# Lcrypto/mod-interleaveavx_multithreads-FAID

Measured on AMD Instinct MI355X. Metric: decoded Gb/s @ 10 iters, 50G-PON LDPC; FER match vs AVX512 ref, higher is better.
Workload: dtype i8

## Files before the change

include/lnsfaid.h:

```cpp
#ifndef LNSFAID_H
#define LNSFAID_H

#include <stddef.h>
#include <stdint.h>

#ifdef __cplusplus
extern "C" {
#endif

#define LNSFAID_GROUP 32

#define LNSFAID_OK 0
#define LNSFAID_E_INVAL (-1)
#define LNSFAID_E_CODE (-2)
#define LNSFAID_E_NOMEM (-3)
#define LNSFAID_E_HIP (-4)
#define LNSFAID_E_NODEVICE (-5)
#define LNSFAID_E_INTERNAL (-6)

typedef struct lnsfaid_code {
    int32_t n_var;
    int32_t n_check;
    int32_t n_edges;
    int32_t z;
// ... 215 lines not shown
int lnsfaid_select_kernel(lnsfaid_ctx* ctx, int32_t rows_per_lane);
int lnsfaid_kernel_rows_per_lane(const lnsfaid_ctx* ctx);

int lnsfaid_select_waves(lnsfaid_ctx* ctx, int32_t waves_per_codeword);
int lnsfaid_kernel_waves(const lnsfaid_ctx* ctx);

#define LNSFAID_MSG_REGISTERS 1
#define LNSFAID_MSG_HBM 2
int lnsfaid_select_message_store(lnsfaid_ctx* ctx, int32_t where);
int lnsfaid_message_store(const lnsfaid_ctx* ctx);

#define LNSFAID_ZERO_SHIFT_ON 1
#define LNSFAID_ZERO_SHIFT_OFF 2
#define LNSFAID_ZERO_SHIFT_LOOP 3
#define LNSFAID_ZERO_SHIFT_STATIC 4
int lnsfaid_select_zero_shift(lnsfaid_ctx* ctx, int32_t mode);
int lnsfaid_zero_shift_groups(const lnsfaid_ctx* ctx, int32_t* groups, int32_t n);
int lnsfaid_code_zero_shift_order(const lnsfaid_code* code, int32_t* groups, int32_t* order);

int lnsfaid_code_bf_walk(const lnsfaid_code* code, int32_t col_weight, uint32_t* full, uint32_t* flipped, uint32_t* fixed, int32_t* info);

int lnsfaid_kernel_residency(lnsfaid_ctx* ctx, int32_t* workgroups_per_cu, int32_t* lds_limit);


int lnsfaid_kernel_time(lnsfaid_ctx* ctx, double* out_ms, uint64_t* out_launches, int32_t reset);

void* lnsfaid_stream(lnsfaid_ctx* ctx);

const char* lnsfaid_strerror(int err);
const char* lnsfaid_last_hip_error(void);
const char* lnsfaid_version(void);

// ... 5 lines not shown
```

mod-interleaveavx_multithreads-faid_amd/csrc/lnsfaid_capi.hip:

```cpp
#include <hip/hip_runtime.h>

#include <dlfcn.h>
#include <rccl/rccl.h>

#include <cstdio>
#include <cstdlib>
#include <cstring>
#include <new>
#include <vector>

#include "lnsfaid_device.h"
#include "lnsfaid_line.h"
#include "lnsfaid_quantise.h"
#include "lnsfaid_swar.h"

extern "C" hipError_t lf_launch_decode(int method, int uniform_w, const LfKernelArgs* args, size_t lds_bytes,
                                       hipStream_t stream);
extern "C" const void* lf_decode_func(int method, int uniform_w);
extern "C" int lf_decode_threads(void);
extern "C" const void* lf_decode4_func(int method, int ef, int rm);
extern "C" int lf_decode4_threads(void);
extern "C" hipError_t lf_launch_decode4(int method, int ef, int rm, const LfKernelArgs* args, size_t lds_bytes, hipStream_t stream);
extern "C" int lf_decode4_rm_layers(void);
extern "C" const void* lf_decode4cw_func(int method, int ef, int rm);
// ... 1 lines not shown
extern "C" const void* lf_decode4p_func(int method, int ef, int rm, int per_codeword);
extern "C" hipError_t lf_launch_decode4p(int method, int ef, int rm, const LfKernelArgs* args, size_t lds_bytes, hipStream_t stream);
extern "C" hipError_t lf_launch_decode4pcw(int method, int ef, int rm, const LfCwArgs* args, size_t lds_bytes, hipStream_t stream);
extern "C" const void* lf_decode4l_func(int method, int ef, int rm);
extern "C" hipError_t lf_launch_decode4l(int method, int ef, int rm, const LfLineArgs* args, size_t lds_bytes, hipStream_t stream);
extern "C" hipError_t lf_launch_unpack_llr4(const uint8_t* d_llr4, int8_t* d_fix, size_t n_values, hipStream_t stream);
extern "C" hipError_t lf_launch_pack_bits(const int8_t* d_decoded, uint32_t* d_bits, size_t n_values, hipStream_t stream);
extern "C" hipError_t lf_launch_count_errors_packed(const uint32_t* d_bits, const uint32_t* d_msg, int n_var, int k_info, size_t n_cw,
                                                    unsigned long long* out, hipStream_t stream);
extern "C" int lf_decode4z_inst(int deg, int zg);
extern "C" const void* lf_decode4z_func(int method);
extern "C" hipError_t lf_launch_decode4z(int method, const LfKernelArgs* args, size_t lds_bytes, hipStream_t stream);
extern "C" int lf_decode4s_matches(const LfDevCode* code);
extern "C" const void* lf_decode4s_func(int method);
extern "C" hipError_t lf_launch_decode4s(int method, const LfKernelArgs* args, size_t lds_bytes, hipStream_t stream);
extern "C" const void* lf_decode5_func(int method);
extern "C" int lf_decode5_threads(void);
extern "C" hipError_t lf_launch_decode5(int method, const LfKernelArgs* args, size_t lds_bytes, hipStream_t stream);
extern "C" hipError_t lf_launch_count_errors(const int8_t* decoded, const int8_t* input_bits, int n_var, int k_info,
                                             size_t n_cw, unsigned long long* out, hipStream_t stream);

extern "C" hipError_t lf_launch_frontend(const uint32_t* d_seeds, const unsigned long long* d_draws, int n_streams, int mod_type,
                                         float sigma_ch, float scale, const int8_t* d_codeword, const int8_t* d_frames, int n_var,
                                         int n_check, int interleave, int fast, int8_t* d_fix, int count_limit,
                                         unsigned long long* d_frame_cnt, hipStream_t stream);
extern "C" hipError_t lf_launch_prefec(const float* d_rx, const int8_t* d_sent, size_t n_groups, int mod_type, int n_var, int n_check,
                                       int interleave, int scope, unsigned long long* d_out, hipStream_t stream);
extern "C" hipError_t lf_launch_prefec_fold(unsigned long long* d_frame_cnt, size_t n_streams, unsigned long long* d_acc, hipStream_t stream);
extern "C" hipError_t lf_launch_capture(const int8_t* d_fix, const int8_t* d_decoded, const int8_t* d_sent, size_t n_groups, int n_var,
                                        int n_check, uint32_t skip, uint32_t cap, uint2* d_cnt, uint32_t* d_slots,
// ... 435 lines not shown
    if (!out || !code || !cfg || max_groups == 0 || max_groups > ((size_t)1 << 24)) return LNSFAID_E_INVAL;
    *out = nullptr;
    lnsfaid_ctx* ctx = new (std::nothrow) lnsfaid_ctx();
    if (!ctx) return LNSFAID_E_NOMEM;
    ctx->device = device;
    ctx->max_groups = max_groups;
    if (const char* e = getenv("LNSFAID_ROWS_PER_LANE"))
        ctx->rows_per_lane = (e[0] == '2') ? 2 : 0;
    if (const char* e = getenv("LNSFAID_WAVES_PER_CODEWORD"))
        ctx->waves_per_cw = (e[0] == '2') ? 2 : 0;
    if (const char* e = getenv("LNSFAID_FRONTEND_EXACT"))
        ctx->fe_exact = (e[0] == '1') ? 1 : 0;
    if (const char* e = getenv("LNSFAID_MSG_STORE"))
        ctx->msg_store = (e[0] == 'h') ? LNSFAID_MSG_HBM : ((e[0] == 'r') ? LNSFAID_MSG_REGISTERS : 0);
    if (const char* e = getenv("LNSFAID_ZERO_SHIFT"))
        ctx->zero_shift = (e[0] == 'o' && e[1] == 'f') ? LNSFAID_ZERO_SHIFT_OFF : (e[0] == 'l' ? LNSFAID_ZERO_SHIFT_LOOP : 0);
    g_live_contexts.fetch_add(1, std::memory_order_relaxed);
    const int rc = create_impl(ctx, code, cfg);
    if (rc) { lnsfaid_destroy(ctx); return rc; }
    ctx->comb_slot = comb_join(ctx);
    *out = ctx;
    return LNSFAID_OK;
}

extern "C" int lnsfaid_set_cfg(lnsfaid_ctx* ctx, const lnsfaid_cfg* cfg)
{
    if (!ctx || !cfg) return LNSFAID_E_INVAL;
    LfDevCfg n;
    int rc = build_cfg(cfg, &n);
    if (rc) return rc;
    rc = check_code_for_method(&ctx->hcode, n.method);
// ... 79 lines not shown
    for (int br = 0; br < ctx->hcode.nbr; ++br)
        if (layer_zero_groups(ctx, br) >= 1) return true;
    return false;
}
static bool use_zero_shift(const lnsfaid_ctx* ctx) { return ctx->zero_shift != LNSFAID_ZERO_SHIFT_OFF && zero_shift_possible(ctx); }

static bool static_layers_possible(const lnsfaid_ctx* ctx)
{
    if (ctx->static_code < 0) ctx->static_code = lf_decode4s_matches(&ctx->hcode);
    return ctx->static_code == 1 && zero_shift_possible(ctx) && lf_decode4s_func(ctx->hcfg.method);
}
static bool use_static_layers(const lnsfaid_ctx* ctx)
{
    return use_zero_shift(ctx) && ctx->zero_shift != LNSFAID_ZERO_SHIFT_LOOP && static_layers_possible(ctx);
}

extern "C" int lnsfaid_select_zero_shift(lnsfaid_ctx* ctx, int32_t mode)
{
    if (!ctx || mode < 0 || mode > LNSFAID_ZERO_SHIFT_STATIC) return LNSFAID_E_INVAL;
    if ((mode == LNSFAID_ZERO_SHIFT_ON || mode == LNSFAID_ZERO_SHIFT_LOOP) && !zero_shift_possible(ctx)) return LNSFAID_E_INVAL;
    if (mode == LNSFAID_ZERO_SHIFT_STATIC && !static_layers_possible(ctx)) return LNSFAID_E_INVAL;
    ctx->zero_shift = mode;
    return LNSFAID_OK;
}

extern "C" int lnsfaid_zero_shift_groups(const lnsfaid_ctx* ctx, int32_t* groups, int32_t n)
{
    if (!ctx || n < 0 || (n > 0 && !groups)) return LNSFAID_E_INVAL;
    const bool on = use_zero_shift(ctx);
    for (int br = 0; br < n; ++br) groups[br] = (on && br < ctx->hcode.nbr) ? layer_zero_groups(ctx, br) : 0;
    return on ? (use_static_layers(ctx) ? 2 : 1) : 0;
}

extern "C" int lnsfaid_code_zero_shift_order(const lnsfaid_code* code, int32_t* groups, int32_t* order)
{
    LfDevCode* dc = new (std::nothrow) LfDevCode;
    if (!dc) return LNSFAID_E_NOMEM;
    const int rc = build_code(code, dc);
    if (rc) { delete dc; return rc; }
    const int nbr = dc->nbr;
    for (int br = 0; br < nbr; ++br) {
        int n_zero = 0;
        while (n_zero < dc->deg[br] && dc->zs4tab[br][n_zero] == 0u) ++n_zero;
        if (groups) groups[br] = n_zero / 4;
        for (int j = 0; order && j < LF_MAX_DEG; ++j) {
            order[br * LF_MAX_DEG + j] = -1;
// ... 43 lines not shown
{
    if (packed) {
        *threads = lf_decode4_threads();
        return lf_decode4p_func(ctx->hcfg.method, ctx->hcfg.ef, use_msg_registers(ctx) ? 1 : 0, rule == LNSFAID_STOP_CODEWORD ? 1 : 0);
    }
    if (rule == LNSFAID_STOP_CODEWORD) {
        *threads = lf_decode4_threads();
        return cw_possible(ctx) ? lf_decode4cw_func(ctx->hcfg.method, ctx->hcfg.ef, use_msg_registers(ctx) ? 1 : 0) : nullptr;
    }
    if (use_kernel5(ctx)) {
        *threads = lf_decode5_threads();
        return lf_decode5_func(ctx->hcfg.method);
    }
    if (use_zero_shift(ctx)) {
        *threads = lf_decode4_threads();
        return use_static_layers(ctx) ? lf_decode4s_func(ctx->hcfg.method) : lf_decode4z_func(ctx->hcfg.method);
    }
    if (use_kernel4(ctx)) {
        *threads = lf_decode4_threads();
        return lf_decode4_func(ctx->hcfg.method, ctx->hcfg.ef, use_msg_registers(ctx) ? 1 : 0);
    }
    *threads = lf_decode_threads();
    return lf_decode_func(ctx->hcfg.method, ctx->hcfg.uniform_w);
}

extern "C" int lnsfaid_select_message_store(lnsfaid_ctx* ctx, int32_t where)
{
    if (!ctx || where < 0 || where > LNSFAID_MSG_HBM) return LNSFAID_E_INVAL;
    if (where == LNSFAID_MSG_REGISTERS && !msg_registers_possible(ctx)) return LNSFAID_E_INVAL;
    ctx->msg_store = where;
// ... 142 lines not shown
    int cur = 0;
    long launch = 0, needed = 0;
    bool done = false;
    while (!done) {
        if (launch >= max_launches) return LNSFAID_E_INTERNAL;
        int chain = launch == 0 ? ctx->predicted_launches : 1;
        if (chain < 1) chain = 1;
        if (chain > LF_MAX_CHAIN) chain = LF_MAX_CHAIN;
        for (int j = 0; j < chain; ++j) {
            a.status_cur = (launch + j == 0 && !status_preloaded) ? nullptr : ctx->d_status[cur];
            a.status_next = ctx->d_status[cur ^ 1];
            a.remaining = ctx->d_remaining + j;
            HIP_TRY(hipEventRecord(ctx->ev_chain[j], ctx->stream));
            if (packed) HIP_TRY(lf_launch_decode4p(ctx->hcfg.method, ctx->hcfg.ef, use_msg_registers(ctx) ? 1 : 0, &a, ctx->lds_bytes, ctx->stream));
            else if (use_kernel5(ctx)) HIP_TRY(lf_launch_decode5(ctx->hcfg.method, &a, ctx->lds_bytes, ctx->stream));
            else if (use_static_layers(ctx)) HIP_TRY(lf_launch_decode4s(ctx->hcfg.method, &a, ctx->lds_bytes, ctx->stream));
            else if (use_zero_shift(ctx)) HIP_TRY(lf_launch_decode4z(ctx->hcfg.method, &a, ctx->lds_bytes, ctx->stream));
            else if (use_kernel4(ctx)) HIP_TRY(lf_launch_decode4(ctx->hcfg.method, ctx->hcfg.ef, use_msg_registers(ctx) ? 1 : 0, &a, ctx->lds_bytes, ctx->stream));
            else HIP_TRY(lf_launch_decode(ctx->hcfg.method, ctx->hcfg.uniform_w, &a, ctx->lds_bytes, ctx->stream));
            cur ^= 1;
        }
        HIP_TRY(hipEventRecord(ctx->ev_chain[chain], ctx->stream));
        HIP_TRY(hipMemcpyAsync(ctx->h_remaining, ctx->d_remaining, (size_t)chain * sizeof(uint32_t), hipMemcpyDeviceToHost, ctx->stream));
        { const int rcw = stream_wait(ctx); if (rcw) return rcw; }
        for (int j = 0; j < chain; ++j) {
            const uint32_t left = ctx->h_remaining[j] - ctx->slot_seen[j];
            ctx->slot_seen[j] = ctx->h_remaining[j];
            float ms = 0.f;
            HIP_TRY(hipEventElapsedTime(&ms, ctx->ev_chain[j], ctx->ev_chain[j + 1]));
            ctx->kernel_ms += ms;
// ... 1620 lines not shown
```

mod-interleaveavx_multithreads-faid_amd/csrc/lnsfaid_swar.h:

```cpp
#ifndef LNSFAID_SWAR_H
#define LNSFAID_SWAR_H

#include <stdint.h>

#if defined(__HIPCC__)
#define SW_DEV 1
#define SW_FN __device__ __forceinline__
#define SW_HD __host__ __device__ __forceinline__
#else
#define SW_DEV 0
#define SW_FN static inline
#define SW_HD static inline
#endif

#define SW_MAX_DEG 24
#ifndef SW_ILP
#define SW_ILP 4
#endif

#if SW_DEV
#define SW_SCHED_FENCE() __builtin_amdgcn_sched_barrier(0)
#else
#define SW_SCHED_FENCE() ((void)0)
#endif
// ... 60 lines not shown
    return k;
#endif
}

#define SW_T2N_LO 0xf900fafbu
#define SW_T2N_HI 0xf8000000u

struct SwK {
    uint32_t c78, c0642, cfc, sel_sign, tt_lo, tt_hi, oh_lo, oh_hi;
    uint32_t cbit[8];
    uint32_t c7f;
    uint32_t c70;
    uint32_t n_lo, n_hi;
    uint32_t c55, c33, c0f;
    uint32_t cm27;
};
SW_FN SwK sw_consts(uint32_t dep = 0u)
{
    SwK k;
    k.c78 = sw_vconst(0x78787878u, dep); k.c0642 = sw_vconst(0x06040200u, dep); k.cfc = sw_vconst(0xfcu, dep);
    k.sel_sign = sw_vconst(0x0b090a08u, dep);
    k.tt_lo = sw_vconst(0x07030100u, dep); k.tt_hi = sw_vconst(0xff3f1f0fu, dep);
    k.oh_lo = sw_vconst(0x08040201u, dep); k.oh_hi = sw_vconst(0x80402010u, dep);
    for (int e = 0; e < 8; ++e) k.cbit[e] = sw_vconst(0x01010101u << e, dep);
    k.c7f = sw_vconst(0x7f7f7f7fu, dep);
    k.c70 = sw_vconst(0x70707070u, dep);
    k.n_lo = sw_vconst(SW_T2N_LO, dep); k.n_hi = sw_vconst(SW_T2N_HI, dep);
    k.c55 = sw_vconst(0x55555555u, dep); k.c33 = sw_vconst(0x33333333u, dep); k.c0f = sw_vconst(0x0f0f0f0fu, dep);
    k.cm27 = sw_vconst(0u - 0x27272727u, dep);
    return k;
}

SW_FN uint32_t sw_mask7(uint32_t x, uint32_t sel_sign) { return sw_perm(x, x << 8, sel_sign); }
#define SW_SEL_SIGN 0x0b090a08u
SW_FN uint64_t sw_shl8x2(uint32_t& a, uint32_t& b)
{
    uint64_t p = ((uint64_t)b << 32) | a;
#if SW_DEV
    asm("" : "+v"(p));
    a = (uint32_t)p; b = (uint32_t)(p >> 32);
    uint64_t r = p << 8;
    asm("" : "+v"(r));
    return r;
#else
// ... 8 lines not shown
    *ma = sw_mask7_lo(a, sh, sel_sign);
    *mb = sw_mask7_hi(b, sh, sel_sign);
}

SW_FN uint32_t sw_popcount7(uint32_t x)
{
    x &= 0x7f7f7f7fu;
    x = x - ((x >> 1) & 0x55555555u);
    x = (x & 0x33333333u) + ((x >> 2) & 0x33333333u);
    return (x + (x >> 4)) & 0x0f0f0f0fu;
}
SW_FN uint32_t sw_therm2num(uint32_t x, uint32_t n_lo, uint32_t n_hi)
{
    const uint32_t a = sw_perm(n_hi, n_lo, x & 0x0f0f0f0fu);
    const uint32_t b = sw_perm(n_hi, n_lo, (x >> 4) & 0x07070707u);
    return a ^ b;
}
SW_FN uint32_t sw_zero_mask(uint32_t x, uint32_t sel_sign) { return ~sw_mask7(x + 0x7f7f7f7fu, sel_sign); }
SW_FN void sw_zero_mask2(uint32_t x, uint32_t y, uint32_t sel_sign, uint32_t* zx, uint32_t* zy)
{
    uint32_t mx, my;
    sw_mask7x2(x + 0x7f7f7f7fu, y + 0x7f7f7f7fu, sel_sign, &mx, &my);
    *zx = ~mx;
    *zy = ~my;
}

SW_FN uint32_t sw_gather4(uint32_t g0, uint32_t g1, uint32_t g2, uint32_t g3)
{
    const uint32_t lo = (g1 << 8) | g0, hi = (g3 << 8) | g2;
    return (hi << 16) | lo;
// ... 265 lines not shown
    SW_MFN uint32_t get(int) const { return 0u; }
    SW_MFN void barrier() const {}
};
#define SW_OWN(j) (WAVES == 1 || (((j) & 1) == WAVE))

template <class Tab>
struct SwTabStatic {
    static constexpr bool value = false;
    static constexpr int nz = 0;
};

#define SW_PAIRS_PASS1 1
#define SW_PAIRS_PASS2 2
#define SW_PAIRS_ROW 4
#define SW_PAIRS_ALL (SW_PAIRS_PASS1 | SW_PAIRS_PASS2 | SW_PAIRS_ROW)
template <int METHOD, int DEG, bool ERA = false, int WAVES = 1, int WAVE = 0, int ZG = 0, int PAIRS = 0, class Tab, class Xch = SwNoXch>
SW_FN SwRow sw_layer_step(const SwLds& lds, const Tab& tab, const SwParams& p, const SwK& K, uint32_t lane, int deg, SwRow cur, bool fresh,
                          uint32_t rowpar, bool lme, uint32_t era_edges = 0u, uint32_t era_plane = 0u, const Xch& xch = Xch())
{
    static_assert(WAVES == 1 || !ERA, "the erasing variant is built for one wave per codeword only");
    static_assert(!ERA || METHOD == 2, "the erasure exists in Decode_FAID only");
    static_assert(ZG == 0 || (DEG > 0 && WAVES == 1 && !ERA && SW_ILP * ZG <= DEG), "rotation-free groups: per-degree, one-wave, non-erasing instances");
    constexpr bool STATIC = SwTabStatic<Tab>::value;
    static_assert(!STATIC || (ZG == 0 && DEG > 0 && WAVES == 1 && !ERA && SwTabStatic<Tab>::nz <= DEG), "static table view: per-degree, one-wave, non-erasing instances");
    constexpr int NZ = STATIC ? SwTabStatic<Tab>::nz : SW_ILP * ZG;
    constexpr int NJ = DEG > 0 ? DEG : SW_MAX_DEG;
    constexpr bool MINSUM = SW_MINSUM(METHOD);
    constexpr bool QUADS = WAVES == 1 && SW_ILP == 4 && DEG > 0;
    constexpr bool NSTREE = WAVES == 1 && SW_ILP == 4;
    constexpr bool EPAIRS = WAVES == 1 && DEG > 0 && SW_ILP % 2 == 0;
    constexpr bool EPAIRS1 = EPAIRS && (PAIRS & SW_PAIRS_PASS1), EPAIRS2 = EPAIRS && (PAIRS & SW_PAIRS_PASS2), RPAIRS = (PAIRS & SW_PAIRS_ROW) != 0;
    const uint32_t c01 = K.cbit[0], c80 = K.cbit[7], c7f = K.c7f, c78 = K.c78, c0642 = K.c0642, cfc = K.cfc, sel_sign = K.sel_sign;
    const uint32_t tid4 = lane << 2;
    uint32_t s4j[NJ], cbj[NJ];
#pragma unroll
    for (int j = 0; j < NJ; ++j) { s4j[j] = (DEG > 0 || j < deg) ? tab.s4(j) : 0u; cbj[j] = (DEG > 0 || j < deg) ? tab.cb256(j) : 0u; }

    const uint32_t c2o = cur.cw & 0x07070707u, c1o = (cur.cw >> 3) & 0x07070707u;
    const uint32_t kp = 0x08080808u - c2o, kn = 0x08080808u + c2o;
    const uint32_t bias = MINSUM ? 0u : 0x06040200u;
    const uint32_t kt_lo = sw_perm(kn, kp, 0x05010400u) + (MINSUM ? 0u : 0x02020000u), kt_hi = sw_perm(kn, kp, 0x07030602u) + (MINSUM ? 0u : 0x06060404u);
    const uint32_t tt_lo = K.tt_lo, tt_hi = K.tt_hi;

    uint32_t padd = 0, psub = 0;
#ifndef SW_EXP_NO_OLDPATCH
    if (!fresh && WAVE == 0) {
        const uint32_t a0 = cur.pa[0] & 0xffffu, a1 = cur.pa[0] >> 16, a2 = cur.pa[1] & 0xffffu, a3 = cur.pa[1] >> 16;
        SW_SCHED_FENCE();
        const uint32_t g0 = lds.rd8(a0), g1 = lds.rd8(a1), g2 = lds.rd8(a2), g3 = lds.rd8(a3);
        const uint32_t mneg = sw_mask7(cur.cw << 1, sel_sign);
        padd = sw_bitop3<SW_TT_SEL>(mneg, c1o, c2o); psub = sw_bitop3<SW_TT_SEL>(mneg, c2o, c1o);
        SW_SCHED_FENCE();
        const uint32_t r = sw_gather4(g0, g1, g2, g3) + padd - psub;
        const uint32_t rh = sw_opaque(r >> 8);
        lds.wr8(a0, r); lds.wr8(a1, rh); lds.wr8(a2, r >> 16); lds.wr8(a3, rh >> 16);
    }
#endif
    if (WAVES == 2) xch.barrier();

    SW_SCHED_FENCE();
    uint32_t tb[NJ], ts[NJ], ms[NJ], ad[NJ], rq[NJ], ld[NJ];
// ... 37 lines not shown
            SW_EDGES(PRE)                                                                                                                \
        }
#define SW_MASK_EXPAND(EPAIRS, DST, SRC)                                                                                                 \
        if (EPAIRS) {                                                                                                                    \
            _Pragma("unroll") for (int g = 0; g < SW_ILP; ++g) {                                                                         \
                const int j = j0 + g;                                                                                                    \
                if (j < NJ) DST(g, j) = (g & 1) ? sw_mask7_hi(SRC(g, j), sh_[g >> 1], sel_sign) : sw_mask7_lo(SRC(g, j), sh_[g >> 1], sel_sign); \
            }                                                                                                                            \
        } else {                                                                                                                         \
            SW_EDGES(DST(g, j) = sw_mask7(SRC(g, j), sel_sign);)                                                                         \
        }
#define SW_P1_TS(g, j) ts[j]
#define SW_P1_MS(g, j) ms[j]
#define SW_P2_MO(g, j) mo[g]
        _Pragma("unroll") for (int g = SW_ILP - 1; g >= 0; --g) { const int j = j0 + g; if (j < NJ && (DEG > 0 || j < deg) && SW_OWN(j)) r_[g] = j < NZ ? ld[j] : sw_alignbyte(ld[j], ld[j], rq[j]); }
        SW_EDGES(x_[g] = (j & 7) ? cur.x[j >> 3] >> (j & 7) : cur.x[j >> 3];)
        SW_EDGES(s_[g] = sw_bitop3<SW_TT_ANDOR>(x_[g], c01, c0642);)
        SW_EDGES(k_[g] = sw_perm(kt_hi, kt_lo, s_[g]);)
        if ((j0 + SW_ILP < NJ ? j0 + SW_ILP : NJ) <= NZ) { _Pragma("unroll") for (int g = SW_ILP - 1; g >= 0; --g) if (j0 + g < NJ) tb[j0 + g] = r_[g] + k_[g]; }
        else { SW_EDGES(tb[j] = r_[g] + k_[g];) }
        if (ERA) {
            SW_EDGES(x_[g] &= c01;)
            SW_EDGES(
                if ((era_edges >> j) & 1u) {
                    uint32_t em = 0, match = 0;
                    _Pragma("unroll") for (int k = 0; k < 4; ++k) {
                        const uint32_t a = ad[j] + ((rq[j] + (uint32_t)k) & 3u);
                        em |= sw_plane_bit(lds, era_plane, a) ? (0xffu << (8 * k)) : 0u;
                        const uint32_t pold = (k & 1) ? cur.pa[k >> 1] >> 16 : cur.pa[k >> 1] & 0xffffu;
                        match |= (!fresh && a == pold) ? (0xffu << (8 * k)) : 0u;
                    }
                    const uint32_t en_true = r_[g] - (padd & match) + (psub & match);
                    const uint32_t neg01 = ~((en_true + 0x08080808u) >> 7) & c01;
// ... 6 lines not shown
            if (WAVES == 2) sx ^= ts[j];                                             \
            else if (j & 1) sx = sw_bitop3<SW_TT_XOR3>(sx, ts[j - 1], ts[j]); else if (j == (DEG > 0 ? DEG : deg) - 1) sx ^= ts[j];)
        if (EPAIRS1) { SW_SX_STAGE }
        SW_MASK_EXPAND(EPAIRS1, SW_P1_MS, SW_P1_TS) }
        SW_EDGES(a_[g] = sw_bitop3<SW_TT_XOR3>(ts[j], c7f, ms[j]);)
        if (METHOD == 0) {
            uint32_t h_[SW_ILP];
            SW_EDGES(i_[g] = sw_bitop3<SW_TT_NANDOR>(ms[j], c01, K.c70);)
            SW_EDGES(a_[g] = (a_[g] + i_[g]) & 0x8f8f8f8fu;)
            SW_EDGES(h_[g] = sw_mask7(a_[g] << 4, sel_sign);)
            SW_EDGES(a_[g] &= 0x87878787u;)
            SW_EDGES(i_[g] = sw_perm(p.nms_t[3], p.nms_t[2], a_[g]);)
            SW_EDGES(u_[g] = sw_perm(p.nms_t[1], p.nms_t[0], a_[g]);)
            SW_EDGES(u_[g] = sw_bitop3<SW_TT_SEL>(h_[g], i_[g], u_[g]);)
        } else {
            SW_EDGES(i_[g] = MINSUM ? sw_bitop3<SW_TT_NANDOR>(ms[j], c01, c78) : sw_bitop3<SW_TT_XNOR_AND>(x_[g], ms[j], c01);)
            SW_EDGES(a_[g] = (MINSUM ? a_[g] + i_[g] : a_[g] + i_[g] + c78) & 0x87878787u;)
            SW_EDGES(u_[g] = sw_perm(tt_hi, tt_lo, a_[g]);)
        }
        if (!EPAIRS1) { SW_SX_STAGE }
        if (QUADS) {
            uint32_t v_[4];
            _Pragma("unroll") for (int g = 0; g < 4; ++g) v_[g] = j0 + g < NJ ? u_[g] : 0xffffffffu;
            sw_min_quad(t1, t2, ta, v_[0], v_[1], v_[2], v_[3], j0);
        } else {
            SW_EDGES(sw_min_edge(t1, t2, ta, u_[g], j);)
        }
    }

    if (WAVES == 2) {
        if (WAVE == 1) {
// ... 4 lines not shown
            const uint32_t o1 = xch.get(0), o2 = xch.get(1);
            ta[0] = t1;
            t2 = sw_bitop3<SW_TT_AND3>(t2, o2, t1 | o1);
            t1 &= o1;
            ta[1] &= xch.get(2); ta[2] &= xch.get(3); ta[3] &= xch.get(4); ta[4] &= xch.get(5);
            sx ^= xch.get(6);
        }
    }
    uint32_t c2n_x = 0, fm_x = 0;
    if (WAVES == 2 && WAVE == 1) {
        xch.barrier();
        c2n_x = xch.get(0); fm_x = xch.get(1);
    }

    const uint32_t n_lo = WAVES == 2 ? SW_T2N_LO : K.n_lo, n_hi = WAVES == 2 ? SW_T2N_HI : K.n_hi;
    const uint32_t min1 = sw_therm2num(t1, n_lo, n_hi), min2 = sw_therm2num(t2, n_lo, n_hi);
    uint32_t c1n, c2n;
    if (METHOD == 0) {
        c2n = min1;
        c1n = min2;
    } else if (SW_OMS(METHOD)) {
        const bool win = p.window && lme;
        const uint32_t w_lo = win ? p.oms_lo[1] : p.oms_lo[0], w_hi = win ? p.oms_hi[1] : p.oms_hi[0];
        c2n = sw_table_pick(rowpar, w_hi, w_lo, p.oms_hi[0], p.oms_lo[0], min1);
        c1n = sw_table_pick(rowpar, w_hi, w_lo, p.oms_hi[0], p.oms_lo[0], min2);
    } else {
        const bool win = (METHOD == 5 || p.ef_tables) && p.window && lme;
        const uint32_t w_lo = win ? p.ef_lo : p.lut_lo, w_hi = win ? p.ef_hi : p.lut_hi;
        c2n = sw_table_pick(rowpar, w_hi, w_lo, p.lut_hi, p.lut_lo, min1);
        c1n = sw_table_pick(rowpar, w_hi, w_lo, p.lut_hi, p.lut_lo, min2);
    }
#if SW_DEV
    asm volatile("" : "+v"(c1n), "+v"(c2n));
// ... 68 lines not shown
    }
    SW_SCHED_FENCE();
    SW_PASS2_STORE(0, en0)
    if (SW_ILP < NJ) { SW_PASS2_ARITH(SW_ILP, en1) SW_PASS2_STORE(SW_ILP, en1) }
    SW_SCHED_FENCE();
    const uint32_t oh8 = sw_perm(K.oh_hi, K.oh_lo, idx & 0x07070707u);
    uint32_t nm3, nm4;
    if (RPAIRS && (DEG == 0 || DEG > 16)) {
        sw_mask7x2(ne7_3, ne7_4, sel_sign, &nm3, &nm4);
        if (DEG == 0 && deg <= 16) nm4 = 0xffffffffu;
        if (DEG == 0 && deg <= 8) nm3 = 0xffffffffu;
    } else {
        nm4 = (DEG == 0 && deg <= 16) ? 0xffffffffu : sw_mask7(ne7_4, sel_sign);
        nm3 = (DEG == 0 && deg <= 8) ? 0xffffffffu : sw_mask7(ne7_3, sel_sign);
    }
    const uint32_t selA = sw_argmin_selector(sw_word_pick(nm3, nm4, cur.x[0], cur.x[1], cur.x[2]), oh8, c7f, c01, c0642);
    if (ERA) xb = selA & c01;
    const uint32_t gb = sw_gather4(gk0, gk1, gk2, gk3);
    uint32_t tbA = gb + sw_perm(kt_hi, kt_lo, selA);
    if (ERA) {
        uint32_t em = 0, match = 0;
#pragma unroll
        for (int k = 0; k < 4; ++k) {
            const uint32_t ik = (idx >> (8 * k)) & 31u;
            if ((era_edges >> ik) & 1u) em |= sw_plane_bit(lds, era_plane, pa[k]) ? (0xffu << (8 * k)) : 0u;
            const uint32_t pold = (k & 1) ? cur.pa[k >> 1] >> 16 : cur.pa[k >> 1] & 0xffffu;
            match |= (!fresh && pa[k] == pold) ? (0xffu << (8 * k)) : 0u;
        }
        const uint32_t en_true = gb - (padd & match) + (psub & match);
        tbA = sw_bitop3<SW_TT_SEL>(em, c80 + bias, tbA);
        xb = sw_bitop3<SW_TT_SEL>(em, ~((en_true + 0x08080808u) >> 7) & c01, xb);
    }
    const uint32_t tsA = MINSUM ? tbA : tbA - (ERA ? (xb | c0642) : selA);
    const uint32_t msA = sw_mask7(tsA, sel_sign);
// ... 60 lines not shown
```

mod-interleaveavx_multithreads-faid_amd/pyabi.py:

```python
import ctypes as C
import os

HERE = os.path.dirname(os.path.abspath(__file__))
LIB_PATH = os.path.join(HERE, "csrc", "liblnsfaid.so")

GROUP = 32
MSG_REGISTERS, MSG_HBM = 1, 2
ZERO_SHIFT_ON, ZERO_SHIFT_OFF, ZERO_SHIFT_LOOP, ZERO_SHIFT_STATIC = 1, 2, 3, 4
STOP_GROUP, STOP_CODEWORD = 0, 1
LINE_HARD, LINE_LLR4 = 0, 1


class Code(C.Structure):
    _fields_ = [
        ("n_var", C.c_int32),
        ("n_check", C.c_int32),
        ("n_edges", C.c_int32),
        ("z", C.c_int32),
        ("puncture_tail", C.c_int32),
        ("nb_degres", C.c_int32),
        ("deg", C.POINTER(C.c_int32)),
        ("deg_rows", C.POINTER(C.c_int32)),
        ("pos_vn", C.POINTER(C.c_uint16)),
    ]
# ... 122 lines not shown
    "lnsfaid_comm_unique_id": (C.c_int, [C.c_void_p]),
    "lnsfaid_comm_init": (C.c_int, [C.c_void_p, C.c_int32, C.c_int32, C.c_void_p]),
    "lnsfaid_comm_attach": (C.c_int, [C.c_void_p, C.c_void_p]),
    "lnsfaid_comm_destroy": (C.c_int, [C.c_void_p]),
    "lnsfaid_allreduce_counters": (C.c_int, [C.c_void_p, C.POINTER(C.c_uint64)]),
    "lnsfaid_select_kernel": (C.c_int, [C.c_void_p, C.c_int32]),
    "lnsfaid_kernel_rows_per_lane": (C.c_int, [C.c_void_p]),
    "lnsfaid_select_waves": (C.c_int, [C.c_void_p, C.c_int32]),
    "lnsfaid_frontend_set_exact": (C.c_int, [C.c_void_p, C.c_int32]),
    "lnsfaid_frontend_fastpath_bounds": (C.c_int, [C.c_void_p, C.POINTER(C.c_double), C.POINTER(C.c_double)]),
    "lnsfaid_kernel_waves": (C.c_int, [C.c_void_p]),
    "lnsfaid_select_message_store": (C.c_int, [C.c_void_p, C.c_int32]),
    "lnsfaid_message_store": (C.c_int, [C.c_void_p]),
    "lnsfaid_select_zero_shift": (C.c_int, [C.c_void_p, C.c_int32]),
    "lnsfaid_zero_shift_groups": (C.c_int, [C.c_void_p, C.POINTER(C.c_int32), C.c_int32]),
    "lnsfaid_code_zero_shift_order": (C.c_int, [C.POINTER(Code), C.POINTER(C.c_int32), C.POINTER(C.c_int32)]),
    "lnsfaid_code_bf_walk": (C.c_int, [C.POINTER(Code), C.c_int32, C.POINTER(C.c_uint32), C.POINTER(C.c_uint32), C.POINTER(C.c_uint32),
                                      C.POINTER(C.c_int32)]),
    "lnsfaid_kernel_residency": (C.c_int, [C.c_void_p, C.POINTER(C.c_int32), C.POINTER(C.c_int32)]),
    "lnsfaid_kernel_time": (C.c_int, [C.c_void_p, C.POINTER(C.c_double), C.POINTER(C.c_uint64), C.c_int32]),
    "lnsfaid_stream": (C.c_void_p, [C.c_void_p]),
    "lnsfaid_strerror": (C.c_char_p, [C.c_int]),
    "lnsfaid_last_hip_error": (C.c_char_p, []),
    "lnsfaid_version": (C.c_char_p, []),
}


def bind(lib, symbols):
    for name, (res, args) in symbols.items():
        fn = getattr(lib, name)
# ... 650 lines not shown

    def select_zero_shift(self, mode):
        self._check(self.lib.lnsfaid_select_zero_shift(self.ctx, mode), "lnsfaid_select_zero_shift")

    def zero_shift_groups(self, n_layers=32):
        zg = (C.c_int32 * n_layers)()
        on = self.lib.lnsfaid_zero_shift_groups(self.ctx, zg, n_layers)
        self._check(min(on, 0), "lnsfaid_zero_shift_groups")
        return on >= 1, list(zg)

    def static_layers(self):
        on = self.lib.lnsfaid_zero_shift_groups(self.ctx, None, 0)
        self._check(min(on, 0), "lnsfaid_zero_shift_groups")
        return on == 2

    def kernel_residency(self):
        wg, lim = C.c_int32(), C.c_int32()
        self._check(self.lib.lnsfaid_kernel_residency(self.ctx, C.byref(wg), C.byref(lim)), "lnsfaid_kernel_residency")
        return wg.value, lim.value

    def kernel_time(self, reset=False):
        ms = C.c_double()
        n = C.c_uint64()
        self._check(self.lib.lnsfaid_kernel_time(self.ctx, C.byref(ms), C.byref(n), 1 if reset else 0), "lnsfaid_kernel_time")
        return ms.value, n.value

    def close(self):
        if self.ctx:
            self.lib.lnsfaid_destroy(self.ctx)
            self.ctx = C.c_void_p()
# ... 7 lines not shown
```

Measured before the change: 87.64.

## Add window-free static-layer decode kernel with specialised first-iteration form

Adds a new decode4w kernel for the static-layer, register-message path. It skips the windowed-min conversion by mapping thermometer minima straight to messages through precomputed permute tables, and it specialises the first iteration so fresh rows skip reading old messages and argmin selection. The kernel is selected by default when static layers apply and no floor threshold is set, and a 'windowed' mode keeps the old kernel available. The risk is a numerical mismatch if the window-free mapping does not match the windowed path exactly, and the extra template instances add code size.

```diff
diff --git a/include/lnsfaid.h b/include/lnsfaid.h
--- a/include/lnsfaid.h
+++ b/include/lnsfaid.h
@@ -253,8 +253,10 @@
 #define LNSFAID_ZERO_SHIFT_OFF 2
 #define LNSFAID_ZERO_SHIFT_LOOP 3
 #define LNSFAID_ZERO_SHIFT_STATIC 4
+#define LNSFAID_ZERO_SHIFT_WINDOWED 5
 int lnsfaid_select_zero_shift(lnsfaid_ctx* ctx, int32_t mode);
 int lnsfaid_zero_shift_groups(const lnsfaid_ctx* ctx, int32_t* groups, int32_t n);
+int lnsfaid_window_free(const lnsfaid_ctx* ctx);
 int lnsfaid_code_zero_shift_order(const lnsfaid_code* code, int32_t* groups, int32_t* order);
 
 int lnsfaid_code_bf_walk(const lnsfaid_code* code, int32_t col_weight, uint32_t* full, uint32_t* flipped, uint32_t* fixed, int32_t* info);
diff --git a/mod-interleaveavx_multithreads-faid_amd/csrc/lnsfaid_capi.hip b/mod-interleaveavx_multithreads-faid_amd/csrc/lnsfaid_capi.hip
--- a/mod-interleaveavx_multithreads-faid_amd/csrc/lnsfaid_capi.hip
+++ b/mod-interleaveavx_multithreads-faid_amd/csrc/lnsfaid_capi.hip
@@ -39,6 +39,8 @@
 extern "C" int lf_decode4s_matches(const LfDevCode* code);
 extern "C" const void* lf_decode4s_func(int method);
 extern "C" hipError_t lf_launch_decode4s(int method, const LfKernelArgs* args, size_t lds_bytes, hipStream_t stream);
+extern "C" const void* lf_decode4w_func(int method);
+extern "C" hipError_t lf_launch_decode4w(int method, const LfKernelArgs* args, size_t lds_bytes, hipStream_t stream);
 extern "C" const void* lf_decode5_func(int method);
 extern "C" int lf_decode5_threads(void);
 extern "C" hipError_t lf_launch_decode5(int method, const LfKernelArgs* args, size_t lds_bytes, hipStream_t stream);
@@ -504,7 +506,8 @@
     if (const char* e = getenv("LNSFAID_MSG_STORE"))
         ctx->msg_store = (e[0] == 'h') ? LNSFAID_MSG_HBM : ((e[0] == 'r') ? LNSFAID_MSG_REGISTERS : 0);
     if (const char* e = getenv("LNSFAID_ZERO_SHIFT"))
-        ctx->zero_shift = (e[0] == 'o' && e[1] == 'f') ? LNSFAID_ZERO_SHIFT_OFF : (e[0] == 'l' ? LNSFAID_ZERO_SHIFT_LOOP : 0);
+        ctx->zero_shift = (e[0] == 'o' && e[1] == 'f') ? LNSFAID_ZERO_SHIFT_OFF
+                          : (e[0] == 'l' ? LNSFAID_ZERO_SHIFT_LOOP : (e[0] == 'w' ? LNSFAID_ZERO_SHIFT_WINDOWED : 0));
     g_live_contexts.fetch_add(1, std::memory_order_relaxed);
     const int rc = create_impl(ctx, code, cfg);
     if (rc) { lnsfaid_destroy(ctx); return rc; }
@@ -614,12 +617,17 @@
 {
     return use_zero_shift(ctx) && ctx->zero_shift != LNSFAID_ZERO_SHIFT_LOOP && static_layers_possible(ctx);
 }
+static bool use_window_free(const lnsfaid_ctx* ctx)
+{
+    return use_static_layers(ctx) && ctx->zero_shift != LNSFAID_ZERO_SHIFT_WINDOWED && ctx->hcfg.floor_iter_thresh < 0 &&
+           lf_decode4w_func(ctx->hcfg.method);
+}
 
 extern "C" int lnsfaid_select_zero_shift(lnsfaid_ctx* ctx, int32_t mode)
 {
-    if (!ctx || mode < 0 || mode > LNSFAID_ZERO_SHIFT_STATIC) return LNSFAID_E_INVAL;
+    if (!ctx || mode < 0 || mode > LNSFAID_ZERO_SHIFT_WINDOWED) return LNSFAID_E_INVAL;
     if ((mode == LNSFAID_ZERO_SHIFT_ON || mode == LNSFAID_ZERO_SHIFT_LOOP) && !zero_shift_possible(ctx)) return LNSFAID_E_INVAL;
-    if (mode == LNSFAID_ZERO_SHIFT_STATIC && !static_layers_possible(ctx)) return LNSFAID_E_INVAL;
+    if ((mode == LNSFAID_ZERO_SHIFT_STATIC || mode == LNSFAID_ZERO_SHIFT_WINDOWED) && !static_layers_possible(ctx)) return LNSFAID_E_INVAL;
     ctx->zero_shift = mode;
     return LNSFAID_OK;
 }
@@ -630,6 +638,12 @@
     const bool on = use_zero_shift(ctx);
     for (int br = 0; br < n; ++br) groups[br] = (on && br < ctx->hcode.nbr) ? layer_zero_groups(ctx, br) : 0;
     return on ? (use_static_layers(ctx) ? 2 : 1) : 0;
+}
+
+extern "C" int lnsfaid_window_free(const lnsfaid_ctx* ctx)
+{
+    if (!ctx) return LNSFAID_E_INVAL;
+    return use_window_free(ctx) ? 1 : 0;
 }
 
 extern "C" int lnsfaid_code_zero_shift_order(const lnsfaid_code* code, int32_t* groups, int32_t* order)
@@ -703,6 +717,7 @@
     }
     if (use_zero_shift(ctx)) {
         *threads = lf_decode4_threads();
+        if (use_window_free(ctx)) return lf_decode4w_func(ctx->hcfg.method);
         return use_static_layers(ctx) ? lf_decode4s_func(ctx->hcfg.method) : lf_decode4z_func(ctx->hcfg.method);
     }
     if (use_kernel4(ctx)) {
@@ -875,6 +890,7 @@
             HIP_TRY(hipEventRecord(ctx->ev_chain[j], ctx->stream));
             if (packed) HIP_TRY(lf_launch_decode4p(ctx->hcfg.method, ctx->hcfg.ef, use_msg_registers(ctx) ? 1 : 0, &a, ctx->lds_bytes, ctx->stream));
             else if (use_kernel5(ctx)) HIP_TRY(lf_launch_decode5(ctx->hcfg.method, &a, ctx->lds_bytes, ctx->stream));
+            else if (use_window_free(ctx)) HIP_TRY(lf_launch_decode4w(ctx->hcfg.method, &a, ctx->lds_bytes, ctx->stream));
             else if (use_static_layers(ctx)) HIP_TRY(lf_launch_decode4s(ctx->hcfg.method, &a, ctx->lds_bytes, ctx->stream));
             else if (use_zero_shift(ctx)) HIP_TRY(lf_launch_decode4z(ctx->hcfg.method, &a, ctx->lds_bytes, ctx->stream));
             else if (use_kernel4(ctx)) HIP_TRY(lf_launch_decode4(ctx->hcfg.method, ctx->hcfg.ef, use_msg_registers(ctx) ? 1 : 0, &a, ctx->lds_bytes, ctx->stream));
diff --git a/mod-interleaveavx_multithreads-faid_amd/csrc/lnsfaid_kernel4w.hip b/mod-interleaveavx_multithreads-faid_amd/csrc/lnsfaid_kernel4w.hip
--- /dev/null
+++ b/mod-interleaveavx_multithreads-faid_amd/csrc/lnsfaid_kernel4w.hip
@@ -0,0 +1,255 @@
+#include <hip/hip_runtime.h>
+
+#define LF4_MAIN_STEP main_step4w
+#define LF4_DIRTY_CHECK(c, lane) dirty4w(lane)
+#include "lnsfaid_rows4.h"
+#include "lnsfaid_static50.h"
+
+static_assert(SW50_LAYERS == LF4_RM_LAYERS, "one register of every message vector per layer");
+
+__device__ __forceinline__ bool dirty4w(int lane)
+{
+    const SwLds lds = SwLds();
+    asm volatile("; lf4w check stage 1");
+    const uint32_t w1 = sw50_row_parity<SW50_CHECK_LAYER>(lds, (uint32_t)lane);
+    if (__ballot((w1 & 0x80808080u) != 0u) != 0ull) return true;
+    asm volatile("; lf4w check stage 2");
+    const uint32_t w0 = sw50_row_parity<0>(lds, (uint32_t)lane);
+    return __ballot((w0 & 0x80808080u) != 0u) != 0ull;
+}
+
+#ifdef LF4W_KEEP_WINDOW
+#define LF4W_BASE 0
+#else
+#define LF4W_BASE SW_FORM_NOWIN
+#endif
+#ifdef LF4W_KEEP_FIRST
+#define LF4W_FRESH 0
+#else
+#define LF4W_FRESH SW_FORM_FRESH
+#endif
+
+template <int METHOD, int FORM, int BR>
+__device__ __forceinline__ void layer4w(const uint32_t (*zsb)[32], SwRegs& R, const SwLds& lds, const SwParams& p, const SwK& K, int lane, bool fresh,
+                                        uint32_t& tabv)
+{
+    typedef Sw50Tab<BR> Tab;
+    asm volatile("; lf4w layer %1" : "+v"(lane) : "n"(BR));
+    uint32_t tabn = 0u;
+    if (BR + 1 < SW50_LAYERS) tabn = zsb[BR + 1][lane & 31];
+    Tab tab;
+    tab.sbv = tabv;
+    const SwRow zero = { { 0u, 0u, 0u }, 0u, { 0u, 0u } };
+    const SwRow cur = (FORM & SW_FORM_FRESH) ? zero : regs_get(R, BR);
+    SwRow st = sw_layer_step<METHOD, Tab::DEG, false, 1, 0, 0, SW_PAIRS_ALL, FORM>(lds, tab, p, K, (uint32_t)lane, Tab::DEG, cur,
+                                                                                  (FORM & SW_FORM_FRESH) ? true : fresh, 0u, false);
+    asm volatile("" : "+v"(st.x[0]), "+v"(st.x[1]), "+v"(st.x[2]), "+v"(st.cw), "+v"(st.pa[0]), "+v"(st.pa[1]));
+    __builtin_amdgcn_sched_barrier(0);
+    regs_put(R, BR, st);
+    __builtin_amdgcn_sched_barrier(0);
+    tabv = tabn;
+}
+
+template <int METHOD, int FORM>
+__device__ __forceinline__ void layers4w(const uint32_t (*zsb)[32], SwRegs& R, const SwLds& lds, const SwParams& p, const SwK& K, int lane, bool fresh,
+                                         uint32_t tabv)
+{
+#define LF4W_LAYER(BR) layer4w<METHOD, FORM, BR>(zsb, R, lds, p, K, lane, fresh, tabv);
+    LF4W_LAYER(0) LF4W_LAYER(1) LF4W_LAYER(2) LF4W_LAYER(3) LF4W_LAYER(4) LF4W_LAYER(5)
+    LF4W_LAYER(6) LF4W_LAYER(7) LF4W_LAYER(8) LF4W_LAYER(9) LF4W_LAYER(10) LF4W_LAYER(11)
+#undef LF4W_LAYER
+}
+
+template <int METHOD, bool ERA, bool RM>
+__device__ __forceinline__ void main_step4w(CCode c, CCfg f, const LfDevCode* gc, SwRow* __restrict__ rows, SwRegs& R, int lane, int it, const uint32_t* sP,
+                                            bool have_par, bool lme, uint32_t era_plane)
+{
+    static_assert(RM && !ERA, "built for the messages-in-registers, non-erasing instances only");
+    (void)c; (void)rows; (void)era_plane; (void)sP; (void)have_par; (void)lme;
+    it = __builtin_amdgcn_readfirstlane(it);
+    SwK K = sw_consts((uint32_t)it);
+    const bool first = (it == 1);
+    const int itx = (it >= 1 && it <= 5) ? it - 1 : 5;
+    SwParams p;
+    p.lut_lo = f->lut_lo[itx][0]; p.lut_hi = f->lut_hi[itx][0];
+    p.ef_lo = f->lut_ef_lo[itx][0]; p.ef_hi = f->lut_ef_hi[itx][0];
+    p.f1 = f->factor_1; p.f2 = f->factor_2;
+    p.window = false;
+    p.ef_tables = f->ef >= 1;
+    if (LF4_OMS(METHOD)) sw_oms_tables(p);
+    {
+        uint32_t tm[4];
+        sw_therm2msg_tables(LF4_OMS(METHOD) ? p.oms_lo[0] : p.lut_lo, LF4_OMS(METHOD) ? p.oms_hi[0] : p.lut_hi, tm);
+#pragma unroll
+        for (int w = 0; w < 4; ++w) K.tm[w] = sw_vconst(tm[w], (uint32_t)it);
+    }
+    const SwLds lds = SwLds();
+    uint32_t z = 0u;
+    asm volatile("" : "+s"(z));
+    const uint32_t (*zsb)[32] = (const uint32_t (*)[32])((const char*)gc->zsbplain + z);
+    const uint32_t tabv = zsb[0][lane & 31];
+    __builtin_amdgcn_sched_barrier(0);
+    if (first) {
+        asm volatile("; lf4w first begin");
+        layers4w<METHOD, LF4W_BASE | LF4W_FRESH>(zsb, R, lds, p, K, lane, true, tabv);
+        asm volatile("; lf4w first end");
+    } else {
+        asm volatile("; lf4w middle begin");
+        layers4w<METHOD, LF4W_BASE>(zsb, R, lds, p, K, lane, false, tabv);
+        asm volatile("; lf4w middle end");
+    }
+}
+
+#define LF4_ON_FRONT prog >= kmax
+#define LF4_CLEAN_STOPS(t) prog >= kmax && !group_passed(a.live, g, prog, t)
+#define LF4_ON_STOP(t) if (RM && prog >= 2) regs_store(R, g_rows, c->nbr, t);
+#define LF4_ON_PASS(t) publish_pass(a.live, cw, prog, t);
+
+template <int METHOD>
+__global__ __launch_bounds__(LF_T4, 2) void lnsfaid_decode4w_kernel(LfKernelArgs a_)
+{
+    constexpr bool RM = true, EF2 = false;
+    LfKernelArgs a = a_;
+    {
+        uint32_t z = 0u;
+        asm volatile("" : "+s"(z));
+        a.code = (const LfDevCode*)((const char*)a_.code + z);
+        a.cfg = (const LfDevCfg*)((const char*)a_.cfg + z);
+    }
+    extern __shared__ __align__(16) unsigned char smem[];
+    CCode c = (CCode)a.code;
+    CCfg f = (CCfg)a.cfg;
+    const int tid = (int)threadIdx.x;
+    const int cw = (int)blockIdx.x;
+    const int N = c->n_var, M = c->n_check, K = c->k_info, nw = c->n_words, pw = c->p_words;
+    uint32_t* sHard0 = (uint32_t*)smem;
+    uint32_t* sHard2 = (uint32_t*)smem + nw;
+    uint32_t* sHard = (uint32_t*)(smem + lf_lds_off_hard(N));
+    uint32_t* sP = (uint32_t*)(smem + lf_lds_off_p(N, nw));
+    int* sStat = (int*)(smem + lf_lds_off_stat(N, nw, pw));
+    int* sRed = sStat + LNSFAID_GROUP;
+
+    const int max_iter = f->max_iter, max_bf = f->max_bf;
+    const int t_bf0 = max_iter + 1;
+    const int t_end = t_bf0 + max_bf;
+
+    const int g = cw >> 5, lane_in_group = cw & 31;
+    const int sv = a.status_cur ? a.status_cur[g * LNSFAID_GROUP + (tid & 31)] : 0;
+    const int my_status = __builtin_amdgcn_readlane(sv, lane_in_group);
+    if (my_status & LF_DONE) {
+        if (tid == 0) a.status_next[cw] = my_status;
+        return;
+    }
+    if (tid == LNSFAID_GROUP) sRed[LF_ZERO_SLOT] = 0;
+    int kmax;
+    {
+        int v = sv & LF_PROG_MASK;
+        v = imax(v, __builtin_amdgcn_update_dpp(0, v, 0x111, 0xf, 0xf, false));
+        v = imax(v, __builtin_amdgcn_update_dpp(0, v, 0x112, 0xf, 0xf, false));
+        v = imax(v, __builtin_amdgcn_update_dpp(0, v, 0x114, 0xf, 0xf, false));
+        v = imax(v, __builtin_amdgcn_update_dpp(0, v, 0x118, 0xf, 0xf, false));
+        v = imax(v, __builtin_amdgcn_update_dpp(0, v, 0x142, 0xa, 0xf, false));
+        kmax = __builtin_amdgcn_readlane(v, 31);
+    }
+    const int all_same = __ballot(sv != my_status) == 0ull;
+    LF_WG_SYNC();
+    int prog = my_status & LF_PROG_MASK;
+
+    uint32_t* g_en = (uint32_t*)(a.st_en + (size_t)cw * (size_t)N);
+    SwRow* g_rows = (SwRow*)(a.st_rows + (size_t)cw * (size_t)(c->nbr * LF_T));
+    uint32_t* g_bits = a.st_bits + (size_t)cw * (size_t)(3 * nw);
+    int8_t* g_out = a.decoded + (size_t)cw * (size_t)N;
+
+    if (prog != 0 && prog == kmax && !all_same) {
+        if (tid == 0) { a.status_next[cw] = my_status; atomicAdd(a.remaining, 1u); }
+        return;
+    }
+
+    if (my_status != 0 && all_same) {
+        if (tid == 0) {
+            a.status_next[cw] = my_status | LF_DONE;
+            if (a.stats && lane_in_group == 0) {
+                lnsfaid_group_stats st;
+                st.iterations = prog <= max_iter ? prog - 1 : max_iter;
+                st.bf_iterations = prog <= max_iter ? 0 : prog - t_bf0;
+                a.stats[g] = st;
+            }
+        }
+        return;
+    }
+
+    bool in_bf = max_bf > 0 && prog >= t_bf0 && prog != 0;
+    LfLaneState ls = { 0, 0, 0, 0 };
+    SwRegs R;
+    if (RM) regs_clear(R);
+
+    if (prog == 0) {
+        LF4_STAGE_INPUT()
+        LF_WG_SYNC();
+        prog = 1;
+    } else if (!in_bf) {
+        copy_in<23>((uint32_t*)smem, g_en, N >> 2, tid);
+        if (RM && prog >= 2) regs_load(R, g_rows, c->nbr, tid);
+        LF_WG_SYNC();
+    } else {
+        copy_in<9>(sHard, g_bits, nw, tid);
+        copy_in<9>(sHard0, g_bits + nw, nw, tid);
+        copy_in<9>(sHard2, g_bits + 2 * nw, nw, tid);
+        ls = a.st_lane[cw];
+        LF_WG_SYNC();
+    }
+
+    bool parked = false;
+    uint32_t pA = 0, pB = 0;
+    if (!in_bf) {
+        LF4_LAYERED_LOOP()
+        LF4_ENTER_BF()
+    }
+    LF4_BF_LOOPS()
+
+    const bool finished = prog >= t_end;
+    if (finished) {
+        if (!in_bf) build_plane4<false>(c, sHard, 0, tid);
+        write_decoded(sHard, g_out, N, tid);
+        if (tid == 0) {
+            a.status_next[cw] = prog | LF_DONE;
+            if (a.stats && lane_in_group == 0) {
+                lnsfaid_group_stats st;
+                st.iterations = prog <= max_iter ? prog - 1 : max_iter;
+                st.bf_iterations = prog <= max_iter ? 0 : prog - t_bf0;
+                a.stats[g] = st;
+            }
+        }
+    } else {
+        if (!in_bf) {
+            copy_out<23>(g_en, (const uint32_t*)smem, N >> 2, tid);
+        } else {
+            copy_out<9>(g_bits, sHard, nw, tid);
+            copy_out<9>(g_bits + nw, sHard0, nw, tid);
+            copy_out<9>(g_bits + 2 * nw, sHard2, nw, tid);
+            if (tid == 0) a.st_lane[cw] = ls;
+        }
+        write_decoded(sHard, g_out, N, tid);
+        if (tid == 0) { a.status_next[cw] = prog; atomicAdd(a.remaining, 1u); }
+    }
+}
+
+extern "C" const void* lf_decode4w_func(int method)
+{
+    switch (method) {
+    case 1: return (const void*)lnsfaid_decode4w_kernel<1>;
+    case 2: return (const void*)lnsfaid_decode4w_kernel<2>;
+    case 3: return (const void*)lnsfaid_decode4w_kernel<3>;
+    case 4: return (const void*)lnsfaid_decode4w_kernel<4>;
+    case 5: return (const void*)lnsfaid_decode4w_kernel<5>;
+    default: return nullptr;
+    }
+}
+
+extern "C" hipError_t lf_launch_decode4w(int method, const LfKernelArgs* args, size_t lds_bytes, hipStream_t stream)
+{
+    const void* fn = lf_decode4w_func(method);
+    if (!fn) return hipErrorInvalidValue;
+    void* kargs[] = { (void*)args };
+    return hipLaunchKernel(fn, dim3((unsigned)args->n_cw), dim3(LF_T4), kargs, lds_bytes, stream);
+}
diff --git a/mod-interleaveavx_multithreads-faid_amd/csrc/lnsfaid_swar.h b/mod-interleaveavx_multithreads-faid_amd/csrc/lnsfaid_swar.h
--- a/mod-interleaveavx_multithreads-faid_amd/csrc/lnsfaid_swar.h
+++ b/mod-interleaveavx_multithreads-faid_amd/csrc/lnsfaid_swar.h
@@ -98,6 +98,7 @@
     uint32_t n_lo, n_hi;
     uint32_t c55, c33, c0f;
     uint32_t cm27;
+    uint32_t tm[4];
 };
 SW_FN SwK sw_consts(uint32_t dep = 0u)
 {
@@ -112,6 +113,7 @@
     k.n_lo = sw_vconst(SW_T2N_LO, dep); k.n_hi = sw_vconst(SW_T2N_HI, dep);
     k.c55 = sw_vconst(0x55555555u, dep); k.c33 = sw_vconst(0x33333333u, dep); k.c0f = sw_vconst(0x0f0f0f0fu, dep);
     k.cm27 = sw_vconst(0u - 0x27272727u, dep);
+    for (int w = 0; w < 4; ++w) k.tm[w] = 0u;
     return k;
 }
 
@@ -150,6 +152,22 @@
 {
     const uint32_t a = sw_perm(n_hi, n_lo, x & 0x0f0f0f0fu);
     const uint32_t b = sw_perm(n_hi, n_lo, (x >> 4) & 0x07070707u);
+    return a ^ b;
+}
+SW_HD void sw_therm2msg_tables(uint32_t lut_lo, uint32_t lut_hi, uint32_t tm[4])
+{
+    const uint32_t c = ~lut_hi & 0xffu;
+    const uint32_t a = lut_lo ^ (c * 0x01010101u);
+    const uint32_t nb = ~lut_hi;
+    tm[0] = (a & 0x0000ffffu) | ((a & 0x00ff0000u) << 8);
+    tm[1] = a & 0xff000000u;
+    tm[2] = c | (nb & 0x0000ff00u) | ((nb & 0x00ff0000u) << 8);
+    tm[3] = nb & 0xff000000u;
+}
+SW_FN uint32_t sw_therm2msg(uint32_t x, const uint32_t tm[4])
+{
+    const uint32_t a = sw_perm(tm[1], tm[0], x & 0x0f0f0f0fu);
+    const uint32_t b = sw_perm(tm[3], tm[2], (x >> 4) & 0x07070707u);
     return a ^ b;
 }
 SW_FN uint32_t sw_zero_mask(uint32_t x, uint32_t sel_sign) { return ~sw_mask7(x + 0x7f7f7f7fu, sel_sign); }
@@ -445,10 +463,15 @@
 #define SW_PAIRS_PASS2 2
 #define SW_PAIRS_ROW 4
 #define SW_PAIRS_ALL (SW_PAIRS_PASS1 | SW_PAIRS_PASS2 | SW_PAIRS_ROW)
-template <int METHOD, int DEG, bool ERA = false, int WAVES = 1, int WAVE = 0, int ZG = 0, int PAIRS = 0, class Tab, class Xch = SwNoXch>
+#define SW_FORM_NOWIN 1
+#define SW_FORM_FRESH 2
+template <int METHOD, int DEG, bool ERA = false, int WAVES = 1, int WAVE = 0, int ZG = 0, int PAIRS = 0, int FORM = 0, class Tab, class Xch = SwNoXch>
 SW_FN SwRow sw_layer_step(const SwLds& lds, const Tab& tab, const SwParams& p, const SwK& K, uint32_t lane, int deg, SwRow cur, bool fresh,
                           uint32_t rowpar, bool lme, uint32_t era_edges = 0u, uint32_t era_plane = 0u, const Xch& xch = Xch())
 {
+    constexpr bool NOWIN = (FORM & SW_FORM_NOWIN) != 0, FRESH = (FORM & SW_FORM_FRESH) != 0;
+    static_assert(FORM == 0 || (WAVES == 1 && !ERA), "iteration forms: one-wave, non-erasing instances");
+    static_assert(!NOWIN || METHOD != 0, "the normalised min-sum rows read no table after the search");
     static_assert(WAVES == 1 || !ERA, "the erasing variant is built for one wave per codeword only");
     static_assert(!ERA || METHOD == 2, "the erasure exists in Decode_FAID only");
     static_assert(ZG == 0 || (DEG > 0 && WAVES == 1 && !ERA && SW_ILP * ZG <= DEG), "rotation-free groups: per-degree, one-wave, non-erasing instances");
@@ -472,10 +495,11 @@
     const uint32_t bias = MINSUM ? 0u : 0x06040200u;
     const uint32_t kt_lo = sw_perm(kn, kp, 0x05010400u) + (MINSUM ? 0u : 0x02020000u), kt_hi = sw_perm(kn, kp, 0x07030602u) + (MINSUM ? 0u : 0x06060404u);
     const uint32_t tt_lo = K.tt_lo, tt_hi = K.tt_hi;
+    const uint32_t k_fresh = 0x08080808u + bias;
 
     uint32_t padd = 0, psub = 0;
 #ifndef SW_EXP_NO_OLDPATCH
-    if (!fresh && WAVE == 0) {
+    if (!FRESH && !fresh && WAVE == 0) {
         const uint32_t a0 = cur.pa[0] & 0xffffu, a1 = cur.pa[0] >> 16, a2 = cur.pa[1] & 0xffffu, a3 = cur.pa[1] >> 16;
         SW_SCHED_FENCE();
         const uint32_t g0 = lds.rd8(a0), g1 = lds.rd8(a1), g2 = lds.rd8(a2), g3 = lds.rd8(a3);
@@ -543,9 +567,13 @@
 #define SW_P1_MS(g, j) ms[j]
 #define SW_P2_MO(g, j) mo[g]
         _Pragma("unroll") for (int g = SW_ILP - 1; g >= 0; --g) { const int j = j0 + g; if (j < NJ && (DEG > 0 || j < deg) && SW_OWN(j)) r_[g] = j < NZ ? ld[j] : sw_alignbyte(ld[j], ld[j], rq[j]); }
-        SW_EDGES(x_[g] = (j & 7) ? cur.x[j >> 3] >> (j & 7) : cur.x[j >> 3];)
-        SW_EDGES(s_[g] = sw_bitop3<SW_TT_ANDOR>(x_[g], c01, c0642);)
-        SW_EDGES(k_[g] = sw_perm(kt_hi, kt_lo, s_[g]);)
+        if (FRESH) {
+            SW_EDGES(x_[g] = 0u; s_[g] = c0642; k_[g] = k_fresh;)
+        } else {
+            SW_EDGES(x_[g] = (j & 7) ? cur.x[j >> 3] >> (j & 7) : cur.x[j >> 3];)
+            SW_EDGES(s_[g] = sw_bitop3<SW_TT_ANDOR>(x_[g], c01, c0642);)
+            SW_EDGES(k_[g] = sw_perm(kt_hi, kt_lo, s_[g]);)
+        }
         if ((j0 + SW_ILP < NJ ? j0 + SW_ILP : NJ) <= NZ) { _Pragma("unroll") for (int g = SW_ILP - 1; g >= 0; --g) if (j0 + g < NJ) tb[j0 + g] = r_[g] + k_[g]; }
         else { SW_EDGES(tb[j] = r_[g] + k_[g];) }
         if (ERA) {
@@ -582,7 +610,8 @@
             SW_EDGES(u_[g] = sw_perm(p.nms_t[1], p.nms_t[0], a_[g]);)
             SW_EDGES(u_[g] = sw_bitop3<SW_TT_SEL>(h_[g], i_[g], u_[g]);)
         } else {
-            SW_EDGES(i_[g] = MINSUM ? sw_bitop3<SW_TT_NANDOR>(ms[j], c01, c78) : sw_bitop3<SW_TT_XNOR_AND>(x_[g], ms[j], c01);)
+            if (FRESH && !MINSUM) { SW_EDGES(i_[g] = sw_bitop3<0x0a>(ms[j], ms[j], c01);) }
+            else { SW_EDGES(i_[g] = MINSUM ? sw_bitop3<SW_TT_NANDOR>(ms[j], c01, c78) : sw_bitop3<SW_TT_XNOR_AND>(x_[g], ms[j], c01);) }
             SW_EDGES(a_[g] = (MINSUM ? a_[g] + i_[g] : a_[g] + i_[g] + c78) & 0x87878787u;)
             SW_EDGES(u_[g] = sw_perm(tt_hi, tt_lo, a_[g]);)
         }
@@ -617,9 +646,12 @@
     }
 
     const uint32_t n_lo = WAVES == 2 ? SW_T2N_LO : K.n_lo, n_hi = WAVES == 2 ? SW_T2N_HI : K.n_hi;
-    const uint32_t min1 = sw_therm2num(t1, n_lo, n_hi), min2 = sw_therm2num(t2, n_lo, n_hi);
+    const uint32_t min1 = NOWIN ? 0u : sw_therm2num(t1, n_lo, n_hi), min2 = NOWIN ? 0u : sw_therm2num(t2, n_lo, n_hi);
     uint32_t c1n, c2n;
-    if (METHOD == 0) {
+    if (NOWIN) {
+        c2n = sw_therm2msg(t1, K.tm);
+        c1n = sw_therm2msg(t2, K.tm);
+    } else if (METHOD == 0) {
         c2n = min1;
         c1n = min2;
     } else if (SW_OMS(METHOD)) {
@@ -718,10 +750,10 @@
         nm4 = (DEG == 0 && deg <= 16) ? 0xffffffffu : sw_mask7(ne7_4, sel_sign);
         nm3 = (DEG == 0 && deg <= 8) ? 0xffffffffu : sw_mask7(ne7_3, sel_sign);
     }
-    const uint32_t selA = sw_argmin_selector(sw_word_pick(nm3, nm4, cur.x[0], cur.x[1], cur.x[2]), oh8, c7f, c01, c0642);
+    const uint32_t selA = FRESH ? c0642 : sw_argmin_selector(sw_word_pick(nm3, nm4, cur.x[0], cur.x[1], cur.x[2]), oh8, c7f, c01, c0642);
     if (ERA) xb = selA & c01;
     const uint32_t gb = sw_gather4(gk0, gk1, gk2, gk3);
-    uint32_t tbA = gb + sw_perm(kt_hi, kt_lo, selA);
+    uint32_t tbA = gb + (FRESH ? k_fresh : sw_perm(kt_hi, kt_lo, selA));
     if (ERA) {
         uint32_t em = 0, match = 0;
 #pragma unroll
diff --git a/mod-interleaveavx_multithreads-faid_amd/pyabi.py b/mod-interleaveavx_multithreads-faid_amd/pyabi.py
--- a/mod-interleaveavx_multithreads-faid_amd/pyabi.py
+++ b/mod-interleaveavx_multithreads-faid_amd/pyabi.py
@@ -6,7 +6,7 @@
 
 GROUP = 32
 MSG_REGISTERS, MSG_HBM = 1, 2
-ZERO_SHIFT_ON, ZERO_SHIFT_OFF, ZERO_SHIFT_LOOP, ZERO_SHIFT_STATIC = 1, 2, 3, 4
+ZERO_SHIFT_ON, ZERO_SHIFT_OFF, ZERO_SHIFT_LOOP, ZERO_SHIFT_STATIC, ZERO_SHIFT_WINDOWED = 1, 2, 3, 4, 5
 STOP_GROUP, STOP_CODEWORD = 0, 1
 LINE_HARD, LINE_LLR4 = 0, 1
 
@@ -160,6 +160,7 @@
     "lnsfaid_message_store": (C.c_int, [C.c_void_p]),
     "lnsfaid_select_zero_shift": (C.c_int, [C.c_void_p, C.c_int32]),
     "lnsfaid_zero_shift_groups": (C.c_int, [C.c_void_p, C.POINTER(C.c_int32), C.c_int32]),
+    "lnsfaid_window_free": (C.c_int, [C.c_void_p]),
     "lnsfaid_code_zero_shift_order": (C.c_int, [C.POINTER(Code), C.POINTER(C.c_int32), C.POINTER(C.c_int32)]),
     "lnsfaid_code_bf_walk": (C.c_int, [C.POINTER(Code), C.c_int32, C.POINTER(C.c_uint32), C.POINTER(C.c_uint32), C.POINTER(C.c_uint32),
                                       C.POINTER(C.c_int32)]),
@@ -840,6 +841,11 @@
         self._check(min(on, 0), "lnsfaid_zero_shift_groups")
         return on == 2
 
+    def window_free(self):
+        on = self.lib.lnsfaid_window_free(self.ctx)
+        self._check(min(on, 0), "lnsfaid_window_free")
+        return on == 1
+
     def kernel_residency(self):
         wg, lim = C.c_int32(), C.c_int32()
         self._check(self.lib.lnsfaid_kernel_residency(self.ctx, C.byref(wg), C.byref(lim)), "lnsfaid_kernel_residency")
```

New measurement: 89.27, median of 6. 1.02x the previous value.
